# luigifcruz/radio-core

Hardware: AMD Instinct MI355X
Metric: IQ Msamples/s through Tuner+WBFM at 1024 channels (higher is better)
Workload: dtype f32

## Files before the change

### radio-core_amd/csrc/fft_kernel.h

```cpp
#pragma once

#include <hip/hip_runtime.h>

#include <cstdio>
#include <cstdlib>
#include <type_traits>

#include "fft_engine.h"
#include "tile_ns.h"

namespace rcfm {
RCFM_NS_OPEN
namespace fftk {

constexpr int W = RCFM_TILE_W;
constexpr int kLogW = W == 16 ? 4 : W == 8 ? 3 : 2;
static_assert((1 << kLogW) == W, "tile width: 4, 8 or 16 lines");
constexpr int kThreads = 256 * W / 16;

__device__ __forceinline__ float2 cmul(float2 a, float2 b) {
    typedef float v2f __attribute__((ext_vector_type(2)));
    v2f A, B, D;
    A.x = a.x; A.y = a.y; B.x = b.x; B.y = b.y;
    asm("v_pk_mul_f32 %0, %1, %2 op_sel:[0,0] op_sel_hi:[0,1]" : "=v"(D) : "v"(A), "v"(B));
// ... 452 lines not shown
    if constexpr (R > 10 || R == 7 || R == 9) dft_nat<R>(v);
}

constexpr int kRowsPitch = W + 1;

template <bool SWZ, bool P17 = true>
__device__ __forceinline__ int lds_slot(int row, int w) {
    if (SWZ && P17) return row * (W + 1) + w;
    return SWZ ? row * W + (w ^ (row & (W - 1))) : row * W + w;
}

template <int R>
__device__ __forceinline__ void twiddle_powers(float2 w1, float2* pw) {
    pw[1] = w1;
#pragma unroll
    for (int q = 2; q < R; ++q) {
        int hb = 1;
        while (hb * 2 <= q) hb *= 2;
        pw[q] = (hb == q) ? cmul(pw[q / 2], pw[q / 2]) : cmul(pw[hb], pw[q - hb]);
    }
}

template <int L, int R, int MT, bool SWZ, int RG, bool P17 = true, bool GTW = false, int ZQ = 0>
__device__ __forceinline__ void stage_lds(float2* tile, const float2* tw, int w, int rg) {
    static_assert(ZQ == 0 || MT == L, "zero rows are declared for the first stage only");
    constexpr int m = MT / R, step = L / MT, rows = L / R, nit = (rows + RG - 1) / RG;
#pragma unroll
    for (int it = 0; it < nit; ++it) {
        const int b = rg + RG * it;
        if ((rows % RG == 0) || b < rows) {
            const int g = b / m, kp = b - g * m;
            const int base = g * MT + kp;
            float2 v[R];
            float2 pw[GTW ? R : 1];
            if constexpr (GTW) pw[0] = tw[kp * step];
#pragma unroll
            for (int q = 0; q < R; ++q) {
                if (ZQ > 0 && q >= ZQ) v[q] = make_float2(0.f, 0.f);
                else v[q] = tile[lds_slot<SWZ, P17>(base + q * m, w)];
            }
            dft_p<R>(v);
            if constexpr (GTW) {
                twiddle_powers<R>(pw[0], pw);
#pragma unroll
                for (int q = 1; q < R; ++q) v[dft_slot<R>(q)] = cmul(v[dft_slot<R>(q)], pw[q]);
            } else {
#pragma unroll
                for (int q = 1; q < R; ++q) v[dft_slot<R>(q)] = cmul(v[dft_slot<R>(q)], tw[q * kp * step]);
            }
#pragma unroll
            for (int q = 0; q < R; ++q) tile[lds_slot<SWZ, P17>(base + q * m, w)] = v[dft_slot<R>(q)];
        }
    }
}

constexpr bool big_tile_pair(int L) { return L > kFftMaxL; }
constexpr bool triple_tile(int L) { return L == 400; }

template <int L, int R0, int R1, int RL, int S>
__device__ __forceinline__ int last_stage_base(int g) {
    if constexpr (S == 2) {
        return g;
    } else if constexpr (S == 3) {
        constexpr int w1 = L / (R0 * RL);
        const int q1 = g / w1, q2 = g - q1 * w1;
        return q1 + R0 * q2;
    } else {
        constexpr int w1 = L / (R0 * RL), w2 = L / (R0 * R1 * RL);
        const int q1 = g / w1, r1 = g - q1 * w1;
        const int q2 = r1 / w2, q3 = r1 - q2 * w2;
        return q1 + R0 * (q2 + R1 * q3);
    }
}

template <int L, int R0, int R1, int R2, int R3, bool ROWS, int T, class LoadOp, class StoreOp>
__global__ __launch_bounds__(T, (big_tile_pair(L) ? 8 : triple_tile(L) ? 6 : T * 16 / W >= 512 ? 4 : 1)) void k_fft_tile(FftPassDev d, LoadOp load,
                                                                                          StoreOp store) {
    constexpr bool BIG = big_tile_pair(L) || triple_tile(L);
    constexpr int S = (R0 > 1) + (R1 > 1) + (R2 > 1) + (R3 > 1);
    static_assert(S >= 2 && R0 * R1 * R2 * R3 == L, "bad radix list");
    constexpr int RL = (S == 2) ? R1 : (S == 3) ? R2 : R3;
    constexpr int m0 = L / R0;
    constexpr int RG = T / W;
    constexpr int nit0 = (m0 + RG - 1) / RG;
    constexpr int nld = ROWS ? (L * W + T - 1) / T : nit0 * R0;
    __shared__ __attribute__((aligned(16))) float2 tile[L * (ROWS && !BIG ? kRowsPitch : W)];
    __shared__ __attribute__((aligned(16))) float2 tw_lds[BIG ? 1 : L];
    const float2* tw = BIG ? d.stage_tw : tw_lds;
    const FftPass& p = d.p;

    const int tid = threadIdx.x;
    const int w = tid & (W - 1), rg = tid >> kLogW;
    const VBlock vb = vblock_hw();
    LineId id;
    BlockPos bp = block_pos(vb);
    id.batch = bp.batch;
    unsigned o = vb.y;
    const unsigned n_o2 = (unsigned)p.n_o2;
    if (p.flat_outer) {
        const unsigned tiles_inner = ((unsigned)p.n_inner + W - 1) / W;
        o = bp.tile / tiles_inner;
        if (o >= (unsigned)(p.n_o1 * p.n_o2)) return;
        bp.tile -= o * tiles_inner;
    }
    id.o1 = n_o2 == 1 ? o : o / n_o2;
    id.o2 = n_o2 == 1 ? 0 : o - (unsigned)id.o1 * n_o2;
    const int i0 = (int)bp.tile * W;
    const int left = (int)p.n_inner - i0;
    const int wvalid = left < W ? left : W;
    const int64_t in_base = (int64_t)id.batch * d.in_batch + id.o1 * p.in_o1 + id.o2 * p.in_o2 +
                            (p.in_t ? (int64_t)(i0 >> 4) * p.in_t + (i0 & 15) : (int64_t)i0 * p.in_i);
    const int64_t out_base = (int64_t)id.batch * d.out_batch + id.o1 * p.out_o1 + id.o2 * p.out_o2 +
                             (p.out_t ? (int64_t)(i0 >> 4) * p.out_t + (i0 & 15) : (int64_t)i0);
    const unsigned in_l = (unsigned)p.in_l, in_i = (unsigned)p.in_i, out_k = (unsigned)p.out_k;

    constexpr int NF = fetch_count<LoadOp>::value;
    constexpr bool HZ = !ROWS && has_half_zones<LoadOp>::value && L % 2 == 0;
    auto zone = [](int q) -> int { return (q + 1) * m0 <= L / 2 ? 0 : (q * m0 > L / 2 ? 2 : 1); };
    float2 v[nld];
    float2 v2[NF >= 2 ? nld : 1];
    float v3[NF == 3 ? nld : 1];
    static_assert(NF <= 2 || !ROWS, "three-fetch load functors: strided passes only");
    if constexpr (ROWS) {
#pragma unroll
        for (int it = 0; it < nld; ++it) {
            int e = tid + T * it;
            if ((L * W) % T != 0) e = e < L * W ? e : 0;
            const int wl = e / L, l = e - wl * L;
            const int wc = wl < wvalid ? wl : 0;
            id.i = i0 + wc;
            v[it] = load.fetch(id, l, in_base, (unsigned)wc * in_i + (unsigned)l);
            if constexpr (NF == 2) v2[it] = load.fetch2(id, l, in_base, (unsigned)wc * in_i + (unsigned)l);
        }
    } else {
        const int wc = w < wvalid ? w : 0;
        id.i = i0 + wc;
#pragma unroll
        for (int it = 0; it < nit0; ++it) {
            int b = rg + RG * it;
            if (m0 % RG != 0) b = b < m0 ? b : 0;
#pragma unroll
            for (int q = 0; q < R0; ++q) {
                const int l = b + q * m0;
                if constexpr (HZ) {
                    const int z = zone(q);
                    if (z == 2) {
                        v[it * R0 + q] = make_float2(0.f, 0.f);
                        if constexpr (NF == 2) v2[it * R0 + q] = make_float2(0.f, 0.f);
                    } else {
                        v[it * R0 + q] = load.fetch(id, l, in_base, (unsigned)l * in_l + (unsigned)wc, z);
                        if constexpr (NF == 2)
                            v2[it * R0 + q] = load.fetch2(id, l, in_base, (unsigned)l * in_l + (unsigned)wc, z);
                    }
                } else {
                    v[it * R0 + q] = load.fetch(id, l, in_base, (unsigned)l * in_l + (unsigned)wc);
                    if constexpr (NF >= 2)
                        v2[it * R0 + q] = load.fetch2(id, l, in_base, (unsigned)l * in_l + (unsigned)wc);
                    if constexpr (NF == 3)
                        v3[it * R0 + q] = load.fetch3(id, l, in_base, (unsigned)l * in_l + (unsigned)wc);
                }
            }
        }
    }
    if constexpr (!BIG)
        for (int e = tid; e < L; e += T) tw_lds[e] = d.stage_tw[e];
    constexpr bool CTX = has_ctx<LoadOp>::value;
    static_assert(!CTX || (!ROWS && NF == 1), "load context: strided single-fetch passes only");
    auto ctx = [&] {
        if constexpr (CTX) return load.prepare(id);
        else return 0;
    }();

    constexpr int rowsL = L / RL, nitL = (rowsL + RG - 1) / RG;
    auto kbase = [](int g) -> int {
        if constexpr (S == 2) {
            return g;
        } else if constexpr (S == 3) {
            constexpr int w1 = L / (R0 * RL);
            const int q1 = g / w1, q2 = g - q1 * w1;
            return q1 + R0 * q2;
        } else {
            constexpr int w1 = L / (R0 * RL), w2 = L / (R0 * R1 * RL);
            const int q1 = g / w1, r1 = g - q1 * w1;
            const int q2 = r1 / w2, q3 = r1 - q2 * w2;
            return q1 + R0 * (q2 + R1 * q3);
        }
    };
    constexpr bool AUX = has_aux<StoreOp>::value;
    float aux[AUX ? nitL * RL : 1];
    if constexpr (AUX) {
        const int wc = w < wvalid ? w : 0;
        id.i = i0 + wc;
#pragma unroll
        for (int it = 0; it < nitL; ++it) {
            int g = rg + RG * it;
            if (rowsL % RG != 0) g = g < rowsL ? g : 0;
            const int kb = kbase(g);
#pragma unroll
            for (int q = 0; q < RL; ++q) {
                const int k = kb + (L / RL) * q;
                aux[it * RL + q] = store.fetch_aux(id, k, out_base, (unsigned)k * out_k + (unsigned)wc);
            }
        }
    }

    if constexpr (ROWS) {
#pragma unroll
        for (int it = 0; it < nld; ++it) {
            const int e = tid + T * it;
            const int wl = e / L, l = e - wl * L;
            id.i = i0 + wl;
            float2 x;
            if constexpr (NF == 2) x = load.post(id, l, v[it], v2[it]);
            else x = load.post(id, l, v[it]);
            if ((L * W) % T == 0 || e < L * W) tile[lds_slot<true, !BIG>(l, wl)] = x;
        }
        __syncthreads();
        stage_lds<L, R0, L, true, RG, !BIG, BIG>(tile, tw, w, rg);
    } else {
        if constexpr (!BIG) __syncthreads();
        id.i = i0 + (w < wvalid ? w : 0);
#pragma unroll
        for (int it = 0; it < nit0; ++it) {
            const int b = rg + RG * it;
            if ((m0 % RG == 0) || b < m0) {
                float2* x = &v[it * R0];
#pragma unroll
                for (int q = 0; q < R0; ++q) {
                    if constexpr (HZ) {
                        if constexpr (NF == 2) {
                            if (zone(q) != 2) x[q] = load.post(id, b + q * m0, x[q], v2[it * R0 + q], zone(q));
                        } else {
                            if (zone(q) != 2) x[q] = load.post(id, b + q * m0, x[q], zone(q));
                        }
                    } else if constexpr (NF == 3) x[q] = load.post(id, b + q * m0, x[q], v2[it * R0 + q], v3[it * R0 + q]);
                    else if constexpr (NF == 2) x[q] = load.post(id, b + q * m0, x[q], v2[it * R0 + q]);
                    else if constexpr (CTX) x[q] = load.post(id, b + q * m0, x[q], ctx);
                    else x[q] = load.post(id, b + q * m0, x[q]);
                }
                dft_p<R0>(x);
                if constexpr (BIG) {
                    float2 pw[R0];
                    twiddle_powers<R0>(tw[b], pw);
#pragma unroll
                    for (int q = 1; q < R0; ++q) x[dft_slot<R0>(q)] = cmul(x[dft_slot<R0>(q)], pw[q]);
                } else {
#pragma unroll
                    for (int q = 1; q < R0; ++q) x[dft_slot<R0>(q)] = cmul(x[dft_slot<R0>(q)], tw[q * b]);
                }
#pragma unroll
                for (int q = 0; q < R0; ++q) tile[lds_slot<false>(b + q * m0, w)] = x[dft_slot<R0>(q)];
            }
        }
    }
    __syncthreads();
    if constexpr (S >= 3) {
        stage_lds<L, R1, L / R0, ROWS, RG, !BIG, BIG>(tile, tw, w, rg);
        __syncthreads();
    }
    if constexpr (S >= 4) {
        stage_lds<L, R2, L / (R0 * R1), ROWS, RG, !BIG, BIG>(tile, tw, w, rg);
        __syncthreads();
    }

    const unsigned f = (unsigned)(id.o1 * p.tw_o1 + id.o2 * p.tw_o2 + (int64_t)(i0 + w) * p.tw_i);
    float2 D = make_float2(1.f, 0.f);
    constexpr bool PTW = !ROWS;
    if constexpr (PTW) D = big_twiddle(d, f * (unsigned)(L / RL));
    id.i = i0 + w;
    const bool lane_ok = w < wvalid;
#pragma unroll
    for (int it = 0; it < nitL; ++it) {
        const int g = rg + RG * it;
        if ((rowsL % RG == 0) || g < rowsL) {
            float2 x[RL];
#pragma unroll
            for (int q = 0; q < RL; ++q) x[q] = tile[lds_slot<ROWS, !BIG>(g * RL + q, w)];
            dft_p<RL>(x);
            const int kb = kbase(g);
            float2 Tw = make_float2(1.f, 0.f);
            if constexpr (PTW) Tw = big_twiddle(d, f * (unsigned)kb);
            if (lane_ok) {
#pragma unroll
                for (int q = 0; q < RL; ++q) {
                    const int k = kb + (L / RL) * q;
                    float2 y = x[dft_slot<RL>(q)];
                    if constexpr (PTW) {
                        y = cmul(y, Tw);
                        Tw = cmul(Tw, D);
                    }
                    if constexpr (AUX) store(id, k, out_base, (unsigned)k * out_k + (unsigned)w, y, aux[it * RL + q]);
                    else store(id, k, out_base, (unsigned)k * out_k + (unsigned)w, y);
                }
            }
        }
    }
}

template <class T, class = void>
struct mid_upper_rows_zero : std::false_type {};
template <class T>
struct mid_upper_rows_zero<T, std::void_t<decltype(T::kUpperRowsZero)>> : std::bool_constant<T::kUpperRowsZero> {};

template <int L, int R0, int R1, int R2, int R3, int T, class LoadOp, class MidOp, class StoreOp>
__global__ __launch_bounds__(T, (T * 16 / W >= 512 ? 4 : 1)) void k_fft_tile2(FftPassDev d1, FftPassDev d2, LoadOp load,
                                                                     MidOp mid, StoreOp store) {
    constexpr int S = (R0 > 1) + (R1 > 1) + (R2 > 1) + (R3 > 1);
    static_assert(S >= 2 && R0 * R1 * R2 * R3 == L, "bad radix list");
    constexpr int RL = (S == 2) ? R1 : (S == 3) ? R2 : R3;
    constexpr int RG = T / W;
    constexpr int nld = (L * W + T - 1) / T;
    constexpr int rowsL = L / RL, nitL = (rowsL + RG - 1) / RG;
    constexpr int kZeroQ = mid_upper_rows_zero<MidOp>::value ? (L / 2) / (L / R0) + 1 : 0;
    constexpr int kZeroFrom = kZeroQ > 0 && kZeroQ < R0 ? kZeroQ * (L / R0) : L;
    __shared__ __attribute__((aligned(16))) float2 tile[L * kRowsPitch];
    __shared__ __attribute__((aligned(16))) float2 tw[L];
    const FftPass& p1 = d1.p;
    const FftPass& p2 = d2.p;
    const int tid = threadIdx.x;
    const int w = tid & (W - 1), rg = tid >> kLogW;

    LineId id;
    const BlockPos bp = block_pos();
    id.batch = bp.batch;
    id.o1 = 0;
    id.o2 = 0;
    const int i0 = (int)bp.tile * W;
    const int left = (int)p1.n_inner - i0;
    const int wvalid = left < W ? left : W;
    const int64_t in_base = (int64_t)id.batch * d1.in_batch + (int64_t)i0 * p1.in_i;
    const int64_t mid_base = (int64_t)id.batch * d1.out_batch + i0;
    const int64_t out_base = (int64_t)id.batch * d2.out_batch + i0;
    const unsigned in_i = (unsigned)p1.in_i, mid_k = (unsigned)p1.out_k, out_k = (unsigned)p2.out_k;

    auto kbase = [](int g) -> int {
        if constexpr (S == 2) {
            return g;
        } else if constexpr (S == 3) {
            constexpr int w1 = L / (R0 * RL);
            const int q1 = g / w1, q2 = g - q1 * w1;
            return q1 + R0 * q2;
        } else {
            constexpr int w1 = L / (R0 * RL), w2 = L / (R0 * R1 * RL);
            const int q1 = g / w1, r1 = g - q1 * w1;
            const int q2 = r1 / w2, q3 = r1 - q2 * w2;
            return q1 + R0 * (q2 + R1 * q3);
        }
    };

    float2 v[nld];
#pragma unroll
    for (int it = 0; it < nld; ++it) {
        int e = tid + T * it;
        if ((L * W) % T != 0) e = e < L * W ? e : 0;
        const int wl = e / L, l = e - wl * L;
        const int wc = wl < wvalid ? wl : 0;
        id.i = i0 + wc;
        v[it] = load.fetch(id, l, in_base, (unsigned)wc * in_i + (unsigned)l);
    }
    float aux[nitL * RL];
    {
        const int wc = w < wvalid ? w : 0;
        id.i = i0 + wc;
#pragma unroll
        for (int it = 0; it < nitL; ++it) {
            int g = rg + RG * it;
            if (rowsL % RG != 0) g = g < rowsL ? g : 0;
            const int kb = kbase(g);
#pragma unroll
            for (int q = 0; q < RL; ++q) {
                const int k = kb + (L / RL) * q;
                aux[it * RL + q] = mid.fetch_aux(id, k, mid_base, (unsigned)k * mid_k + (unsigned)wc);
            }
        }
    }
    for (int e = tid; e < L; e += T) tw[e] = d1.stage_tw[e];

#pragma unroll
    for (int it = 0; it < nld; ++it) {
        const int e = tid + T * it;
        const int wl = e / L, l = e - wl * L;
        id.i = i0 + wl;
        float2 x = load.post(id, l, v[it]);
        if ((L * W) % T == 0 || e < L * W) tile[lds_slot<true>(l, wl)] = x;
    }
    lds_barrier();
    stage_lds<L, R0, L, true, RG>(tile, tw, w, rg);
    lds_barrier();
    if constexpr (S >= 3) {
        stage_lds<L, R1, L / R0, true, RG>(tile, tw, w, rg);
        lds_barrier();
    }
    if constexpr (S >= 4) {
        stage_lds<L, R2, L / (R0 * R1), true, RG>(tile, tw, w, rg);
        lds_barrier();
    }

    id.i = i0 + w;
    float2 xr[nitL * RL];
#pragma unroll
    for (int it = 0; it < nitL; ++it) {
        const int g = rg + RG * it;
        if ((rowsL % RG == 0) || g < rowsL) {
#pragma unroll
            for (int q = 0; q < RL; ++q) xr[it * RL + q] = tile[lds_slot<true>(g * RL + q, w)];
            dft_p<RL>(&xr[it * RL]);
        }
    }
    lds_barrier();
#pragma unroll
    for (int it = 0; it < nitL; ++it) {
        const int g = rg + RG * it;
        if ((rowsL % RG == 0) || g < rowsL) {
            const int kb = kbase(g);
#pragma unroll
            for (int q = 0; q < RL; ++q) {
                const int k = kb + (L / RL) * q;
                if constexpr (mid_upper_rows_zero<MidOp>::value) {
                    if ((L / RL) * q > L / 2) {
                        if ((L / RL) * q < kZeroFrom) tile[lds_slot<true>(k, w)] = make_float2(0.f, 0.f);
                        continue;
                    }
                }
                float2 y = mid(id, k, xr[it * RL + dft_slot<RL>(q)], aux[it * RL + q]);
                tile[lds_slot<true>(k, w)] = y;
            }
        }
    }
    lds_barrier();

    stage_lds<L, R0, L, true, RG, true, false, kZeroQ>(tile, tw, w, rg);
    lds_barrier();
    if constexpr (S >= 3) {
        stage_lds<L, R1, L / R0, true, RG>(tile, tw, w, rg);
        lds_barrier();
    }
    if constexpr (S >= 4) {
        stage_lds<L, R2, L / (R0 * R1), true, RG>(tile, tw, w, rg);
        lds_barrier();
    }
    const bool lane_ok = w < wvalid;
    const unsigned f = (unsigned)((int64_t)(i0 + w) * p2.tw_i);
    const float2 D = big_twiddle(d2, f * (unsigned)(L / RL));
#pragma unroll
    for (int it = 0; it < nitL; ++it) {
        const int g = rg + RG * it;
        if ((rowsL % RG == 0) || g < rowsL) {
            float2 x[RL];
#pragma unroll
            for (int q = 0; q < RL; ++q) x[q] = tile[lds_slot<true>(g * RL + q, w)];
            dft_p<RL>(x);
            const int kb = kbase(g);
            float2 Tw = big_twiddle(d2, f * (unsigned)kb);
            if (lane_ok) {
#pragma unroll
                for (int q = 0; q < RL; ++q) {
                    const int k = kb + (L / RL) * q;
                    const float2 y = cmul(x[dft_slot<RL>(q)], Tw);
                    Tw = cmul(Tw, D);
                    store(id, k, out_base, (unsigned)k * out_k + (unsigned)w, y);
                }
            }
        }
    }
}

template <int L, int R0, int R1, int R2, int R3, int T, class LoadOp, class MidOp, class StoreOp>
__global__ __launch_bounds__(T, (T * 16 / W >= 512 ? 4 : 1)) void k_fft_tile2_pair(FftPassDev d1, FftPassDev d2, LoadOp load,
                                                                          MidOp mid, StoreOp store, int count) {
    constexpr int S = (R0 > 1) + (R1 > 1) + (R2 > 1) + (R3 > 1);
    static_assert(S >= 2 && R0 * R1 * R2 * R3 == L, "bad radix list");
    constexpr int RL = (S == 2) ? R1 : (S == 3) ? R2 : R3;
    constexpr int RG = T / W;
    constexpr int nld = (L * W + T - 1) / T;
    constexpr int rowsL = L / RL, nitL = (rowsL + RG - 1) / RG;
    __shared__ __attribute__((aligned(16))) float2 tile[L * kRowsPitch];
    __shared__ __attribute__((aligned(16))) float2 tw[L];
    const FftPass& p1 = d1.p;
    const FftPass& p2 = d2.p;
    const int tid = threadIdx.x;
    const int w = tid & (W - 1), rg = tid >> kLogW;

    LineId id;
    const BlockPos bp = block_pos();
    id.batch = bp.batch;
    id.o1 = 0;
    id.o2 = 0;
    const int c0 = 2 * (int)bp.batch;
    const bool has1 = c0 + 1 < count;
    const int c1 = has1 ? c0 + 1 : c0;
    const int i0 = (int)bp.tile * W;
    const int left = (int)p1.n_inner - i0;
    const int wvalid = left < W ? left : W;
    const int64_t in_base = (int64_t)id.batch * d1.in_batch + (int64_t)i0 * p1.in_i;
    const int blk16 = mid.blk16;
    const int64_t mid_tile = blk16 ? (int64_t)(i0 >> 4) * blk16 + (i0 & 15) : (int64_t)i0;
    const int64_t mid_base0 = (int64_t)c0 * (blk16 ? mid.stride : d1.out_batch) + mid_tile;
    const int64_t mid_base1 = (int64_t)c1 * (blk16 ? mid.stride : d1.out_batch) + mid_tile;
    const int64_t out_base0 = (int64_t)c0 * d2.out_batch + i0;
    const int64_t out_base1 = (int64_t)c1 * d2.out_batch + i0;
    const unsigned in_i = (unsigned)p1.in_i, mid_k = blk16 ? 16u : (unsigned)p1.out_k, out_k = (unsigned)p2.out_k;
    const int wc = w < wvalid ? w : 0;

    auto lane_off = [&](int it) -> unsigned {
        int g = rg + RG * it;
        if (rowsL % RG != 0) g = g < rowsL ? g : 0;
        return (unsigned)last_stage_base<L, R0, R1, RL, S>(g) * mid_k + (unsigned)wc;
    };
    auto q_off = [&](int q) -> int64_t { return (int64_t)((L / RL) * q) * mid_k; };

    float2 v[nld];
#pragma unroll
    for (int it = 0; it < nld; ++it) {
        int e = tid + T * it;
        if ((L * W) % T != 0) e = e < L * W ? e : 0;
        const int wl = e / L, l = e - wl * L;
        const int wcl = wl < wvalid ? wl : 0;
        id.i = i0 + wcl;
        v[it] = load.fetch(id, l, in_base, (unsigned)wcl * in_i + (unsigned)l);
    }
    for (int e = tid; e < L; e += T) tw[e] = d1.stage_tw[e];
#pragma unroll
    for (int it = 0; it < nld; ++it) {
        const int e = tid + T * it;
        const int wl = e / L, l = e - wl * L;
        id.i = i0 + wl;
        const float2 x = load.post(id, l, v[it]);
        if ((L * W) % T == 0 || e < L * W) tile[lds_slot<true>(l, wl)] = x;
    }
    lds_barrier();
    stage_lds<L, R0, L, true, RG>(tile, tw, w, rg);
    lds_barrier();
    if constexpr (S >= 3) {
        stage_lds<L, R1, L / R0, true, RG>(tile, tw, w, rg);
        lds_barrier();
    }
    if constexpr (S >= 4) {
        stage_lds<L, R2, L / (R0 * R1), true, RG>(tile, tw, w, rg);
        lds_barrier();
    }

    using In0 = decltype(mid.fetch0(mid_base0, mid_base1, 0u));
    In0 a0[nitL * RL];
#pragma unroll
    for (int it = 0; it < nitL; ++it)
#pragma unroll
        for (int q = 0; q < RL; ++q)
            a0[it * RL + q] = mid.fetch0(mid_base0 + q_off(q), mid_base1 + q_off(q), lane_off(it));

    id.i = i0 + w;
    using Keep = typename MidOp::Keep;
    float2 u0[nitL * RL];
    Keep keep[nitL * RL];
#pragma unroll
    for (int it = 0; it < nitL; ++it) {
        const int g = rg + RG * it;
        if ((rowsL % RG == 0) || g < rowsL) {
            float2 x[RL];
#pragma unroll
            for (int q = 0; q < RL; ++q) x[q] = tile[lds_slot<true>(g * RL + q, w)];
            dft_p<RL>(x);
#pragma unroll
            for (int q = 0; q < RL; ++q)
                u0[it * RL + q] = mid.first(x[dft_slot<RL>(q)], a0[it * RL + q], keep[it * RL + q]);
        }
        __builtin_amdgcn_sched_barrier(0);
    }
    lds_barrier();
#pragma unroll
    for (int it = 0; it < nitL; ++it) {
        const int g = rg + RG * it;
        if ((rowsL % RG == 0) || g < rowsL) {
            const int kb = last_stage_base<L, R0, R1, RL, S>(g);
#pragma unroll
            for (int q = 0; q < RL; ++q) tile[lds_slot<true>(kb + (L / RL) * q, w)] = u0[it * RL + q];
        }
    }
    lds_barrier();

    const unsigned f = (unsigned)((int64_t)(i0 + w) * p2.tw_i);
    const float2 D = big_twiddle(d2, f * (unsigned)(L / RL));
    const bool lane_ok = w < wvalid;
    auto second_transform = [&](int64_t out_base) {
        stage_lds<L, R0, L, true, RG>(tile, tw, w, rg);
        lds_barrier();
        if constexpr (S >= 3) {
            stage_lds<L, R1, L / R0, true, RG>(tile, tw, w, rg);
            lds_barrier();
        }
        if constexpr (S >= 4) {
            stage_lds<L, R2, L / (R0 * R1), true, RG>(tile, tw, w, rg);
            lds_barrier();
        }
#pragma unroll
        for (int it = 0; it < nitL; ++it) {
            const int g = rg + RG * it;
            if ((rowsL % RG == 0) || g < rowsL) {
                float2 x[RL];
#pragma unroll
                for (int q = 0; q < RL; ++q) x[q] = tile[lds_slot<true>(g * RL + q, w)];
                dft_p<RL>(x);
                const int kb = last_stage_base<L, R0, R1, RL, S>(g);
                float2 Tw = big_twiddle(d2, f * (unsigned)kb);
                if (lane_ok) {
#pragma unroll
                    for (int q = 0; q < RL; ++q) {
                        const int k = kb + (L / RL) * q;
                        const float2 y = cmul(x[dft_slot<RL>(q)], Tw);
                        Tw = cmul(Tw, D);
                        store(id, k, out_base, (unsigned)k * out_k + (unsigned)w, y);
                    }
                }
            }
        }
    };

    float a1[nitL * RL];
#pragma unroll
    for (int it = 0; it < nitL; ++it)
#pragma unroll
        for (int q = 0; q < RL; ++q) a1[it * RL + q] = mid.fetch1(mid_base1 + q_off(q), lane_off(it));

    second_transform(out_base0);
    if (!has1) return;
    lds_barrier();
#pragma unroll
    for (int it = 0; it < nitL; ++it) {
        const int g = rg + RG * it;
        if ((rowsL % RG == 0) || g < rowsL) {
            const int kb = last_stage_base<L, R0, R1, RL, S>(g);
#pragma unroll
            for (int q = 0; q < RL; ++q) {
                const int k = kb + (L / RL) * q;
                tile[lds_slot<true>(k, w)] = mid.second(keep[it * RL + q], a1[it * RL + q]);
            }
        }
    }
    lds_barrier();
    second_transform(out_base1);
}

template <int L, int R0, int R1, int R2, int R3, int L2, int Q0, int Q1, int Q2, int T, class LoadOp, class WinOp, class StoreOp>
__global__ __launch_bounds__(T, (T * 16 / W >= 512 ? 4 : 1)) void k_fft_tile2_decim(FftPassDev d1, FftPassDev d2, LoadOp load,
                                                                           WinOp win, StoreOp store) {
    constexpr int S = (R0 > 1) + (R1 > 1) + (R2 > 1) + (R3 > 1);
    static_assert(S >= 2 && R0 * R1 * R2 * R3 == L, "bad radix list");
    constexpr int S2 = (Q0 > 1) + (Q1 > 1) + (Q2 > 1);
    static_assert(S2 >= 2 && Q0 * Q1 * Q2 == L2 && L2 % 2 == 0 && L2 < L, "bad short transform");
    constexpr int RL = (S == 2) ? R1 : (S == 3) ? R2 : R3;
    constexpr int QL = (S2 == 2) ? Q1 : Q2;
    constexpr int RG = T / W;
    constexpr int nld = (L * W + T - 1) / T;
    constexpr int rowsL = L / RL, nitL = (rowsL + RG - 1) / RG;
    constexpr int rows2 = L2 / QL;
    static_assert(rows2 <= RG, "short transform: one sweep");
    constexpr bool REG = S == 2 && nitL == 1 && Q0 == 4 && L2 == 4 * rowsL && RL >= 5 && L % L2 == 0;
    constexpr int nwin = REG ? 4 : (L2 * W + T - 1) / T;
    __shared__ __attribute__((aligned(16))) float2 tile[L * kRowsPitch];
    __shared__ __attribute__((aligned(16))) float2 tw[L];
    const FftPass& p1 = d1.p;
    const FftPass& p2 = d2.p;
    const int tid = threadIdx.x;
    const int w = tid & (W - 1), rg = tid >> kLogW;

    LineId id;
    const BlockPos bp = block_pos();
    id.batch = bp.batch;
    id.o1 = 0;
    id.o2 = 0;
    const int i0 = (int)bp.tile * W;
    const int left = (int)p1.n_inner - i0;
    const int wvalid = left < W ? left : W;
    const int64_t in_base = (int64_t)id.batch * d1.in_batch + (int64_t)i0 * p1.in_i;
    const int64_t out_base = (int64_t)id.batch * d2.out_batch + i0;
    const unsigned in_i = (unsigned)p1.in_i, out_k = (unsigned)p2.out_k;

    float2 v[nld];
#pragma unroll
    for (int it = 0; it < nld; ++it) {
        int e = tid + T * it;
        if ((L * W) % T != 0) e = e < L * W ? e : 0;
        const int wl = e / L, l = e - wl * L;
        const int wcl = wl < wvalid ? wl : 0;
        id.i = i0 + wcl;
        v[it] = load.fetch(id, l, in_base, (unsigned)wcl * in_i + (unsigned)l);
    }
    float wgt[nwin];
    if constexpr (REG) {
        const int g = rg < rowsL ? rg : 0;
#pragma unroll
        for (int q = 0; q < 4; ++q) wgt[q] = win.weight(id, g + rowsL * q, i0 + (w < wvalid ? w : 0));
    } else {
#pragma unroll
        for (int it = 0; it < nwin; ++it) {
            int e = tid + T * it;
            if ((L2 * W) % T != 0) e = e < L2 * W ? e : 0;
            const int wl = e & (W - 1);
            wgt[it] = win.weight(id, e >> kLogW, i0 + (wl < wvalid ? wl : 0));
        }
    }
    const unsigned f = (unsigned)((int64_t)(i0 + w) * p2.tw_i);
    const int kb2 = last_stage_base<L2, Q0, Q1, QL, S2>(rg < rows2 ? rg : 0);
    const float2 seedD = big_twiddle_seed(d2, f * (unsigned)rows2);
    const float2 seedT = big_twiddle_seed(d2, f * (unsigned)kb2);
    float2 tw2 = make_float2(0.f, 0.f);
    if constexpr (REG && S2 == 3) {
        static_assert(L2 <= T, "short stage table: one entry per thread");
        tw2 = d2.stage_tw[tid < L2 ? tid : 0];
    }
    for (int e = tid; e < L; e += T) tw[e] = d1.stage_tw[e];
#pragma unroll
    for (int it = 0; it < nld; ++it) {
        const int e = tid + T * it;
        const int wl = e / L, l = e - wl * L;
        id.i = i0 + wl;
        const float2 x = load.post(id, l, v[it]);
        if ((L * W) % T == 0 || e < L * W) tile[lds_slot<true>(l, wl)] = x;
    }
    lds_barrier();
    stage_lds<L, R0, L, true, RG>(tile, tw, w, rg);
    lds_barrier();
    if constexpr (S >= 3) {
        stage_lds<L, R1, L / R0, true, RG>(tile, tw, w, rg);
        lds_barrier();
    }
    if constexpr (S >= 4) {
        stage_lds<L, R2, L / (R0 * R1), true, RG>(tile, tw, w, rg);
        lds_barrier();
    }

    float2 xr[nitL * RL];
#pragma unroll
    for (int it = 0; it < nitL; ++it) {
        const int g = rg + RG * it;
        if ((rowsL % RG == 0) || g < rowsL) {
#pragma unroll
            for (int q = 0; q < RL; ++q) xr[it * RL + q] = tile[lds_slot<true>(g * RL + q, w)];
            dft_p<RL>(&xr[it * RL]);
        }
    }
    if constexpr (REG) {
        float2 y[4];
        if (rg < rowsL) {
            y[0] = xr[dft_slot<RL>(0)];
            y[1] = xr[dft_slot<RL>(1)];
            y[2] = xr[dft_slot<RL>(RL - 2)];
            y[3] = xr[dft_slot<RL>(RL - 1)];
            const bool first = rg == 0 && i0 + w == 0;
            if (first) y[2] = cadd(y[2], xr[dft_slot<RL>(2)]);
#pragma unroll
            for (int q = 0; q < 4; ++q) y[q] = make_float2(y[q].x * wgt[q], y[q].y * wgt[q]);
            if (first) {
                id.i = 0;
                win.dc_bin(id, y[0]);
            }
#pragma unroll
            for (int q = 0; q < 4; ++q) y[q] = make_float2(y[q].y, y[q].x);
            dft4(y[0], y[1], y[2], y[3]);
#pragma unroll
            for (int q = 1; q < 4; ++q) y[q] = cmul(y[q], tw[(L / L2) * q * rg]);
        }
        lds_barrier();
        if (rg < rowsL) {
#pragma unroll
            for (int q = 0; q < 4; ++q) tile[lds_slot<true>(rg + rowsL * q, w)] = y[q];
        }
        if constexpr (S2 == 3) {
            if (tid < L2) tw[tid] = tw2;
        }
        lds_barrier();
    } else {
        lds_barrier();
#pragma unroll
        for (int it = 0; it < nitL; ++it) {
            const int g = rg + RG * it;
            if ((rowsL % RG == 0) || g < rowsL) {
                const int kb = last_stage_base<L, R0, R1, RL, S>(g);
#pragma unroll
                for (int q = 0; q < RL; ++q) {
                    if ((L / RL) * q > L2 / 2 && (L / RL) * (q + 1) <= L - L2 / 2) continue;
                    const int k = kb + (L / RL) * q;
                    int l = -1;
                    if (k < L2 / 2) l = k;
                    else if (k >= L - L2 / 2) l = k - (L - L2);
                    else if (k == L2 / 2) l = L2;
                    if (l >= 0) tile[lds_slot<true>(l, w)] = xr[it * RL + dft_slot<RL>(q)];
                }
            }
        }
        for (int e = tid; e < L2; e += T) tw[e] = d2.stage_tw[e];
        lds_barrier();

#pragma unroll
        for (int it = 0; it < nwin; ++it) {
            const int e = tid + T * it;
            if ((L2 * W) % T == 0 || e < L2 * W) {
                const int l = e >> kLogW, wl = e & (W - 1);
                float2 x = tile[lds_slot<true>(l, wl)];
                if (l == L2 / 2 && i0 + wl == 0) {
                    const float2 y = tile[lds_slot<true>(L2, wl)];
                    x = make_float2(x.x + y.x, x.y + y.y);
                }
                x = make_float2(x.x * wgt[it], x.y * wgt[it]);
                if (l == 0 && i0 + wl == 0) {
                    id.i = 0;
                    win.dc_bin(id, x);
                }
                tile[lds_slot<true>(l, wl)] = make_float2(x.y, x.x);
            }
        }
        lds_barrier();

        stage_lds<L2, Q0, L2, true, RG>(tile, tw, w, rg);
        lds_barrier();
    }
    if constexpr (S2 == 3) {
        stage_lds<L2, Q1, L2 / Q0, true, RG>(tile, tw, w, rg);
        lds_barrier();
    }
    id.i = i0 + w;
    if (rg < rows2) {
        float2 x[QL];
#pragma unroll
        for (int q = 0; q < QL; ++q) x[q] = tile[lds_slot<true>(rg * QL + q, w)];
        dft_p<QL>(x);
        const float2 D = big_twiddle(d2, f * (unsigned)rows2, seedD);
        float2 Tw = big_twiddle(d2, f * (unsigned)kb2, seedT);
        if (w < wvalid) {
#pragma unroll
            for (int q = 0; q < QL; ++q) {
                const int k = kb2 + rows2 * q;
                const float2 y = cmul(x[dft_slot<QL>(q)], Tw);
                Tw = cmul(Tw, D);
                store(id, k, out_base, (unsigned)k * out_k + (unsigned)w, y);
            }
        }
    }
}


__device__ __forceinline__ float2 stream_load(const float2* p) { return *p; }

__device__ __forceinline__ void stream_store(float2* p, float2 v) {
    if constexpr (W == 16) {
        using v2 = __attribute__((ext_vector_type(2))) float;
        v2 t;
        t.x = v.x;
        t.y = v.y;
        __builtin_nontemporal_store(t, reinterpret_cast<v2*>(p));
    } else {
        *p = v;
    }
}

template <bool SWAP>
struct LoadPlainT {
    const float2* in;
    __device__ __forceinline__ float2 fetch(const LineId&, int, int64_t base, unsigned off) const {
        return stream_load(in + base + off);
    }
    __device__ __forceinline__ float2 post(const LineId&, int, float2 v) const {
        return SWAP ? make_float2(v.y, v.x) : v;
    }
};

__device__ __forceinline__ float2 iq_bits(unsigned raw) { return make_float2(__uint_as_float(raw), 0.f); }

struct LoadIq16 {
    const uint32_t* in;
    __device__ __forceinline__ float2 fetch(const LineId&, int, int64_t base, unsigned off) const {
        return iq_bits(in[base + off]);
    }
    __device__ __forceinline__ float2 post(const LineId&, int, float2 v) const {
        const unsigned raw = __float_as_uint(v.x);
        return make_float2((float)(int16_t)(raw & 0xffffu) * 0x1p-15f, (float)(int16_t)(raw >> 16) * 0x1p-15f);
    }
};

struct LoadIq8 {
    const uint16_t* in;
    __device__ __forceinline__ float2 fetch(const LineId&, int, int64_t base, unsigned off) const {
// ... 255 lines not shown
```

Measured before the change: 34440.

## Fuse first stage of second FFT into registers after mid op in tile2 kernels

For the L=500 single kernel and the L=480 pair kernel, the mid operator output is fed straight into the first radix stage of the second transform while still in registers, with its twiddles applied there. This removes one LDS write/read round trip and a stage_lds pass with its barriers. The 480 pair path also reorders the remaining radices to 6·10·8. Twiddle seeds are computed earlier so their latency overlaps other work. The cost is higher register pressure and more specialised code paths chosen by compile-time macros.

Result: no change. 34780 (median of 6 runs) (+1.0%).

```diff
diff --git a/radio-core_amd/csrc/fft_kernel.h b/radio-core_amd/csrc/fft_kernel.h
--- a/radio-core_amd/csrc/fft_kernel.h
+++ b/radio-core_amd/csrc/fft_kernel.h
@@ -778,6 +778,14 @@
 template <class T>
 struct mid_upper_rows_zero<T, std::void_t<decltype(T::kUpperRowsZero)>> : std::bool_constant<T::kUpperRowsZero> {};
 
+#ifndef RCFM_MID_REGISTERS
+#define RCFM_MID_REGISTERS 2
+#endif
+#ifndef RCFM_PAIR_MID_480
+#define RCFM_PAIR_MID_480 10, 8
+#endif
+constexpr int pair_mid_radix(int which, int q1, int q2) { return which == 1 ? q1 : q2; }
+
 template <int L, int R0, int R1, int R2, int R3, int T, class LoadOp, class MidOp, class StoreOp>
 __global__ __launch_bounds__(T, (T * 16 / W >= 512 ? 4 : 1)) void k_fft_tile2(FftPassDev d1, FftPassDev d2, LoadOp load,
                                                                      MidOp mid, StoreOp store) {
@@ -789,6 +797,8 @@
     constexpr int rowsL = L / RL, nitL = (rowsL + RG - 1) / RG;
     constexpr int kZeroQ = mid_upper_rows_zero<MidOp>::value ? (L / 2) / (L / R0) + 1 : 0;
     constexpr int kZeroFrom = kZeroQ > 0 && kZeroQ < R0 ? kZeroQ * (L / R0) : L;
+    constexpr bool MID = (RCFM_MID_REGISTERS & 1) != 0 && L == 500 && S == 2 && R0 == 25 && RL == 20 && nitL == 1 &&
+                         L / R0 <= RG && mid_upper_rows_zero<MidOp>::value;
     __shared__ __attribute__((aligned(16))) float2 tile[L * kRowsPitch];
     __shared__ __attribute__((aligned(16))) float2 tw[L];
     const FftPass& p1 = d1.p;
@@ -850,6 +860,12 @@
             }
         }
     }
+    [[maybe_unused]] float2 seedD = make_float2(0.f, 0.f), seedT = make_float2(0.f, 0.f);
+    if constexpr (MID) {
+        const unsigned f2 = (unsigned)((int64_t)(i0 + w) * p2.tw_i);
+        seedD = big_twiddle_seed(d2, f2 * (unsigned)(L / R0));
+        seedT = big_twiddle_seed(d2, f2 * (unsigned)(rg < L / R0 ? rg : 0));
+    }
     for (int e = tid; e < L; e += T) tw[e] = d1.stage_tw[e];
 
 #pragma unroll
@@ -882,6 +898,46 @@
             for (int q = 0; q < RL; ++q) xr[it * RL + q] = tile[lds_slot<true>(g * RL + q, w)];
             dft_p<RL>(&xr[it * RL]);
         }
+    }
+    if constexpr (MID) {
+        constexpr int Q0 = RL, QL = R0, m2 = L / Q0, rows2 = L / QL;
+        float2 y[Q0];
+        if (rg < rowsL) {
+#pragma unroll
+            for (int q = 0; q < Q0; ++q) {
+                if ((L / RL) * q > L / 2) y[q] = make_float2(0.f, 0.f);
+                else y[q] = mid(id, rg + (L / RL) * q, xr[dft_slot<RL>(q)], aux[q]);
+            }
+            dft_p<Q0>(y);
+#pragma unroll
+            for (int q = 1; q < Q0; ++q) y[dft_slot<Q0>(q)] = cmul(y[dft_slot<Q0>(q)], tw[q * rg]);
+        }
+        lds_barrier();
+        if (rg < rowsL) {
+#pragma unroll
+            for (int q = 0; q < Q0; ++q) tile[lds_slot<true>(rg + m2 * q, w)] = y[dft_slot<Q0>(q)];
+        }
+        lds_barrier();
+        const bool lane_ok = w < wvalid;
+        const unsigned f = (unsigned)((int64_t)(i0 + w) * p2.tw_i);
+        const float2 D = big_twiddle(d2, f * (unsigned)rows2, seedD);
+        if (rg < rows2) {
+            float2 x[QL];
+#pragma unroll
+            for (int q = 0; q < QL; ++q) x[q] = tile[lds_slot<true>(rg * QL + q, w)];
+            dft_p<QL>(x);
+            float2 Tw = big_twiddle(d2, f * (unsigned)rg, seedT);
+            if (lane_ok) {
+#pragma unroll
+                for (int q = 0; q < QL; ++q) {
+                    const int k = rg + rows2 * q;
+                    const float2 y2 = cmul(x[dft_slot<QL>(q)], Tw);
+                    Tw = cmul(Tw, D);
+                    store(id, k, out_base, (unsigned)k * out_k + (unsigned)w, y2);
+                }
+            }
+        }
+        return;
     }
     lds_barrier();
 #pragma unroll
@@ -950,6 +1006,10 @@
     constexpr int RG = T / W;
     constexpr int nld = (L * W + T - 1) / T;
     constexpr int rowsL = L / RL, nitL = (rowsL + RG - 1) / RG;
+    constexpr bool MID = (RCFM_MID_REGISTERS & 2) != 0 && L == 480 && S == 3 && R0 == 10 && R1 == 8 && RL == 6;
+    constexpr int Q0 = RL, Q1 = MID ? pair_mid_radix(1, RCFM_PAIR_MID_480) : R1, QL = MID ? pair_mid_radix(2, RCFM_PAIR_MID_480) : R0;
+    static_assert(!MID || Q0 * Q1 * QL == L, "RCFM_PAIR_MID_480: middle and last radix of 480 = 6 . Q1 . QL");
+    constexpr int rows2 = L / QL, nit2 = (rows2 + RG - 1) / RG;
     __shared__ __attribute__((aligned(16))) float2 tile[L * kRowsPitch];
     __shared__ __attribute__((aligned(16))) float2 tw[L];
     const FftPass& p1 = d1.p;
@@ -1028,6 +1088,11 @@
     using Keep = typename MidOp::Keep;
     float2 u0[nitL * RL];
     Keep keep[nitL * RL];
+    [[maybe_unused]] auto first_stage_twiddle = [&](float2* u, int g) {
+        const int b = last_stage_base<L, R0, R1, RL, S>(g);
+#pragma unroll
+        for (int q = 1; q < RL; ++q) u[dft_slot<RL>(q)] = cmul(u[dft_slot<RL>(q)], tw[q * b]);
+    };
 #pragma unroll
     for (int it = 0; it < nitL; ++it) {
         const int g = rg + RG * it;
@@ -1042,6 +1107,26 @@
         }
         __builtin_amdgcn_sched_barrier(0);
     }
+    [[maybe_unused]] float2 seedD = make_float2(0.f, 0.f);
+    [[maybe_unused]] float2 seedT[nit2];
+    if constexpr (MID) {
+        const unsigned f2 = (unsigned)((int64_t)(i0 + w) * p2.tw_i);
+        seedD = big_twiddle_seed(d2, f2 * (unsigned)rows2);
+#pragma unroll
+        for (int it = 0; it < nit2; ++it) {
+            int g = rg + RG * it;
+            if (rows2 % RG != 0) g = g < rows2 ? g : 0;
+            seedT[it] = big_twiddle_seed(d2, f2 * (unsigned)last_stage_base<L, Q0, Q1, QL, S>(g));
+        }
+#pragma unroll
+        for (int it = 0; it < nitL; ++it) {
+            const int g = rg + RG * it;
+            if ((rowsL % RG == 0) || g < rowsL) {
+                dft_p<RL>(&u0[it * RL]);
+                first_stage_twiddle(&u0[it * RL], g);
+            }
+        }
+    }
     lds_barrier();
 #pragma unroll
     for (int it = 0; it < nitL; ++it) {
@@ -1049,10 +1134,79 @@
         if ((rowsL % RG == 0) || g < rowsL) {
             const int kb = last_stage_base<L, R0, R1, RL, S>(g);
 #pragma unroll
-            for (int q = 0; q < RL; ++q) tile[lds_slot<true>(kb + (L / RL) * q, w)] = u0[it * RL + q];
+            for (int q = 0; q < RL; ++q)
+                tile[lds_slot<true>(kb + (L / RL) * q, w)] = u0[it * RL + (MID ? dft_slot<RL>(q) : q)];
         }
     }
     lds_barrier();
+
+    if constexpr (MID) {
+        const unsigned f = (unsigned)((int64_t)(i0 + w) * p2.tw_i);
+        const bool lane_ok = w < wvalid;
+        const float2 D = big_twiddle(d2, f * (unsigned)rows2, seedD);
+        float2 TwB[nit2];
+#pragma unroll
+        for (int it = 0; it < nit2; ++it) {
+            int g = rg + RG * it;
+            if (rows2 % RG != 0) g = g < rows2 ? g : 0;
+            TwB[it] = big_twiddle(d2, f * (unsigned)last_stage_base<L, Q0, Q1, QL, S>(g), seedT[it]);
+        }
+        auto second_rest = [&](int64_t out_base) {
+            stage_lds<L, Q1, L / Q0, true, RG>(tile, tw, w, rg);
+            lds_barrier();
+#pragma unroll
+            for (int it = 0; it < nit2; ++it) {
+                const int g = rg + RG * it;
+                if ((rows2 % RG == 0) || g < rows2) {
+                    float2 x[QL];
+#pragma unroll
+                    for (int q = 0; q < QL; ++q) x[q] = tile[lds_slot<true>(g * QL + q, w)];
+                    dft_p<QL>(x);
+                    const int kb = last_stage_base<L, Q0, Q1, QL, S>(g);
+                    float2 Tw = TwB[it];
+                    if (lane_ok) {
+#pragma unroll
+                        for (int q = 0; q < QL; ++q) {
+                            const int k = kb + rows2 * q;
+                            const float2 y = cmul(x[dft_slot<QL>(q)], Tw);
+                            Tw = cmul(Tw, D);
+                            store(id, k, out_base, (unsigned)k * out_k + (unsigned)w, y);
+                        }
+                    }
+                }
+            }
+        };
+        second_rest(out_base0);
+        if (!has1) return;
+        float a1[nitL * RL];
+#pragma unroll
+        for (int it = 0; it < nitL; ++it)
+#pragma unroll
+            for (int q = 0; q < RL; ++q) a1[it * RL + q] = mid.fetch1(mid_base1 + q_off(q), lane_off(it));
+#pragma unroll
+        for (int it = 0; it < nitL; ++it) {
+            const int g = rg + RG * it;
+            if ((rowsL % RG == 0) || g < rowsL) {
+#pragma unroll
+                for (int q = 0; q < RL; ++q) u0[it * RL + q] = mid.second(keep[it * RL + q], a1[it * RL + q]);
+                dft_p<RL>(&u0[it * RL]);
+                first_stage_twiddle(&u0[it * RL], g);
+            }
+        }
+        lds_barrier();
+#pragma unroll
+        for (int it = 0; it < nitL; ++it) {
+            const int g = rg + RG * it;
+            if ((rowsL % RG == 0) || g < rowsL) {
+                const int kb = last_stage_base<L, R0, R1, RL, S>(g);
+#pragma unroll
+                for (int q = 0; q < RL; ++q) tile[lds_slot<true>(kb + (L / RL) * q, w)] = u0[it * RL + dft_slot<RL>(q)];
+            }
+        }
+        lds_barrier();
+        second_rest(out_base1);
+        return;
+    }
 
     const unsigned f = (unsigned)((int64_t)(i0 + w) * p2.tw_i);
     const float2 D = big_twiddle(d2, f * (unsigned)(L / RL));
```
